# coolo/rl-6-nimmt

Hardware: AMD Instinct MI355X
Metric: env-steps/sec at 65536 concurrent 4-player games, 1/2/4/8 MI355X (higher is better)
Workload: dtype u32; 1 GPU; config2: 65536 x 4-player DrunkHamster self-play per GPU, one episode (10 env-steps) per launch, numpy-MT RNG, int8 obs + actions + rewards + done emitted; games_per_gpu=65536, players=4, env_steps_per_launch=655360, rng=numpy, obs=True, parallelism=dp1 (independent game shards, no data-path collective), launches_per_call=4

## Files before the change

include/sechs.h:

```cpp
#ifndef SECHS_H
#define SECHS_H
#include <stddef.h>
#include <stdint.h>

#ifdef __cplusplus
extern "C" {
#endif

typedef struct sn_env sn_env;

typedef enum {
    SN_OK = 0,
    SN_EINVAL = 1,
    SN_EHIP = 2,
    SN_ENOMEM = 3,
    SN_EUNSUPPORTED = 4,
    SN_ERNG = 5,
} sn_status;

enum {
    SN_RNG_PHILOX = 0,
    SN_RNG_NUMPY_MT = 1,
};

enum { SN_I8 = 1, SN_I16 = 2, SN_I32 = 3, SN_I64 = 4, SN_F32 = 5 };

enum {
    SN_AUTO_RESET = 1,
    SN_NO_SUMMARIES = 2,
};

const char* sn_last_error(void);
const char* sn_version(void);

sn_status sn_create(sn_env** out, int device, int64_t num_games, int num_players, int num_cards, uint64_t seed,
                    uint64_t game_offset, int rng_mode);
sn_status sn_destroy(sn_env* env);
sn_status sn_info(const sn_env* env, int64_t* num_games, int* num_players, int* num_cards, int* rng_mode);

sn_status sn_reset(sn_env* env, const uint8_t* decks, void* stream);

sn_status sn_reset_to(sn_env* env, const int8_t* board, const int8_t* hands, void* stream);

sn_status sn_step(sn_env* env, const int32_t* actions, int32_t* rewards, uint8_t* done, int32_t* invalid, int flags,
                  void* stream);

sn_status sn_rollout(sn_env* env, int steps, int32_t* rewards, uint8_t* done, uint8_t* actions, int8_t* obs,
                     int obs_stride, int flags, void* stream);

sn_status sn_obs(sn_env* env, void* obs, int dtype, int obs_stride, int flags, void* stream);
sn_status sn_hands(sn_env* env, int8_t* hands, void* stream);
sn_status sn_board(sn_env* env, int8_t* board, void* stream);
sn_status sn_scores(sn_env* env, int32_t* scores, void* stream);
sn_status sn_results(sn_env* env, int32_t* sum_results, int32_t* episodes, void* stream);
sn_status sn_clear_results(sn_env* env, void* stream);

sn_status sn_mt_get(sn_env* env, int64_t game, uint32_t* key_host, int32_t* pos_host);
sn_status sn_mt_set(sn_env* env, int64_t game, const uint32_t* key_host, int32_t pos);
sn_status sn_philox_counter(sn_env* env, int64_t game, uint64_t* counter_host);

enum { SN_OPT_RING_WORDS = 1, SN_OPT_CHUNK_STEPS = 2, SN_OPT_PIPELINE = 3, SN_OPT_TIMING = 4, SN_OPT_PIPE_GPW = 5,
       SN_OPT_PIPE_LEAD = 6, SN_OPT_PLAY_SPLIT = 7, SN_OPT_PLAY_QUAD = 8, SN_OPT_TWIST_ROUND = 9,
       SN_OPT_TWIST_EVERY = 10, SN_OPT_PIPE_FUSED = 11, SN_OPT_TWIST_SKIP = 12, SN_OPT_PIPE_DEC = 13,
       SN_OPT_TWIST_DEPTH = 14 };
sn_status sn_set_option(sn_env* env, int option, int value);
sn_status sn_pipe_errors(sn_env* env, uint32_t* count);
sn_status sn_kernel_times(sn_env* env, float* play_ms, float* ahead_ms, int32_t* n);
sn_status sn_kernel_times_dec(sn_env* env, float* play_ms, float* ahead_ms, float* decode_ms, int32_t* n);
sn_status sn_debug_phases(uint64_t* out, int n);
sn_status sn_debug_puct_phases(uint64_t* out, int n);
sn_status sn_debug_pipe_words(sn_env* env, int what, int slot, uint32_t* out);
sn_status sn_debug_failures(uint32_t* count, uint32_t* first_line, int selftest);

sn_status sn_step1(sn_env* env, const int32_t* actions_host, int32_t* out_host, int flags);
sn_status sn_reset1(sn_env* env, const uint32_t* key_host, int32_t pos, uint32_t* key_out_host, int32_t* pos_out,
                    int32_t* out_host, int flags);

sn_status sn_league_config(sn_env* env, int num_agents, int min_players, int max_players);
sn_status sn_league_rollout(sn_env* env, int steps, int32_t* rewards, uint8_t* done, uint8_t* actions, int8_t* obs,
                            int obs_stride, int32_t* records, void* stream);
sn_status sn_league_seats(sn_env* env, uint32_t* out, void* stream);

enum { SN_AGENT_RANDOM = 0, SN_AGENT_MCS = 1, SN_AGENT_EXTERNAL = 2 };
sn_status sn_league_agents(sn_env* env, const int32_t* kinds_host, const int32_t* mc_per_card_host,
                           const int32_t* mc_max_host);
sn_status sn_league_step(sn_env* env, const int32_t* actions, int32_t* rewards, int32_t* played, int32_t* records,
                         int32_t* invalid, int32_t* status, void* stream);
sn_status sn_elo_replay(const int32_t* records_host, int64_t num_games, int max_players, int num_agents, double elo_k,
                        double* elos_host);


sn_status sn_mcs_memorize(sn_env* env, uint32_t* avail, int mcs_num_cards, void* stream);

sn_status sn_mcs_rollouts(sn_env* env, const uint32_t* avail, int rollouts, uint64_t seed, uint32_t decision_step,
                          int32_t* sums, void* stream);
sn_status sn_mcs_rollouts_ex(sn_env* env, const uint32_t* avail, int rollouts, uint64_t seed, uint32_t decision_step,
                             int32_t* sums, int32_t* playouts, void* stream);

sn_status sn_mcs_choose(sn_env* env, const int32_t* sums, int32_t* actions, void* stream);

sn_status sn_mcs_play_exact(sn_env* env, uint32_t mcs_seats, int mc_per_card, int mc_max, int32_t* actions,
                            int32_t* rewards, int32_t* status, void* stream);

sn_status sn_mcs_decide_exact(int device, int64_t num_decisions, int num_players, const int8_t* board,
                              const int8_t* hand, const uint32_t* avail, int mc_per_card, int mc_max,
                              uint32_t* mt_keys, int32_t* mt_pos, int32_t* actions, int32_t* sums, int32_t* counts,
                              void* stream);

typedef struct {
    uint32_t seats_mask;
    int n;
    int puct_root;
    double c_puct;
    uint64_t seed;
    uint32_t step;
    uint32_t rollout;
    const uint32_t* avail;
// ... 56 lines not shown
```

rl-6-nimmt_amd/csrc/sechs_env.hip:

```cpp
#include <hip/hip_runtime.h>

#include <cmath>
#include <cstdio>
#include <cstdlib>
#include <cstring>
#include <new>
#include <string>
#include <type_traits>

#define SECHS_DEBUG_HERE
#include "sechs_state.h"

using namespace sechs;

__global__ void k_seed(DevState s) {
    const int64_t g = (int64_t)blockIdx.x * blockDim.x + threadIdx.x;
    if (g >= s.B) return;
    if (s.rng_mode == RNG_NUMPY_MT) {
        uint32_t* st = s.mt + g * kMtN;
        uint32_t v = (uint32_t)(s.seed + s.game_offset + (uint64_t)g);
        st[0] = v;
        for (int i = 1; i < kMtN; i++) {
            v = 1812433253u * (v ^ (v >> 30)) + (uint32_t)i;
            st[i] = v;
// ... 467 lines not shown
}

enum {
    PH_PROLOGUE = 0, PH_OBS, PH_DRAW, PH_RESOLVE, PH_STORE, PH_DEAL, PH_EPILOGUE, PH_HANDS, PH_APPLY, PH_B1, PH_B2,
    PR_DRAWS, PR_B1, PR_TARGETS, PR_APPLY, PR_HANDS, PR_DRAWS2, PR_B2, PR_STORE, PR_SPARE, PH_N
};
#ifdef SECHS_PHASE_PROF
__device__ unsigned long long g_phase[PH_N + 2];
struct PhaseProf {
    uint64_t t, acc[PH_N];
    __device__ __forceinline__ void start() {
        t = __builtin_readcyclecounter();
#pragma unroll
        for (int k = 0; k < PH_N; k++) acc[k] = 0ull;
    }
    __device__ __forceinline__ void mark(int k) {
        const uint64_t n = __builtin_readcyclecounter();
        acc[k] += n - t;
        t = n;
    }
    __device__ __forceinline__ void flush(int lane, int role = 0) {
        if (lane == 0) {
#pragma unroll
            for (int k = 0; k < PH_N; k++)
                if (acc[k]) atomicAdd(&g_phase[k], (unsigned long long)acc[k]);
            atomicAdd(&g_phase[PH_N + role], 1ull);
        }
    }
};
#else
struct PhaseProf {
    __device__ __forceinline__ void start() {}
    __device__ __forceinline__ void mark(int) {}
    __device__ __forceinline__ void flush(int, int = 0) {}
};
#endif

constexpr int kPlayPrefetch = 2;

struct PlayArgs {
    int steps, flags, obs_stride, wave_lds;
    int ring_lds;
    int pipe_cin, pipe_cout, pipe_t;
    int vec_out;
    const int32_t* actions;
    int32_t* rewards;
    uint8_t* done;
    uint8_t* actions_out;
    int8_t* obs;
    int32_t* invalid;
    int32_t* league_rec;
    int step0;
    int n0;
    int drec0, drec1;
};

template <int N, class R>
struct StreamSrc {
    R& rng;
    ByteBuf& buf;
    uint8_t* deck;
    __device__ __forceinline__ void draws(const Game<N>& G, int, uint32_t kp, bool lg, uint32_t (&idx)[N]) {
        if (lg && !__all(kp == (uint32_t)N)) {
#pragma unroll
            for (int p = 0; p < N; p++) idx[p] = ((uint32_t)p < kp) ? rng_interval(rng, buf, G.n - 1u) : 0u;
        } else {
            rng_draws<N>(rng, buf, G.n - 1u, idx);
        }
    }
    __device__ __forceinline__ uint32_t league(const DevState& s) { return league_draw(rng, buf, s.lg_K, s.lg_lo, s.lg_hi); }
    __device__ __forceinline__ void deal(const DevState& s, Game<N>& G, PhaseProf& pp) {
        shuffle_targets(rng, buf, deck + kDeckStride, s.C);
        pp.mark(PH_DEAL);
        for (int i = 0; i < s.C; i += 4) *(uint32_t*)(deck + i) = (uint32_t)i * 0x01010101u + 0x03020100u;
        shuffle_apply(deck, deck + kDeckStride, s.C);
        pp.mark(PH_APPLY);
        deal_from_deck<N>(deck, s.C, G);
#pragma unroll
        for (int p = 0; p < N; p++) SN_DASSERT(hand_strict(G.hand[p]) && hand_len(G.hand[p]) == (uint32_t)kHand);
    }
};

constexpr int kDecWords = 4 * kDecQuads;

__device__ __forceinline__ uint32_t dec_u16(const uint32_t (&w)[kDecWords], int base, int t) {
    uint32_t v = 0u;
#pragma unroll
    for (int k = 0; k < 5; k++) v = (t >> 1 == k) ? w[base + k] : v;
    return (t & 1) ? (v >> 16) : (v & 0xFFFFu);
}

template <int N>
struct DecSrc {
    uint32_t A[kDecWords];
    uint32_t B1[11];
    int phi;

    __device__ __forceinline__ void load(const DevState& s, const PlayArgs& a, int64_t g, bool cross) {
        phi = a.n0;
        const u32x4* ra = s.drec + (int64_t)a.drec0 * kDecQuads * s.B + g;
#pragma unroll
        for (int q = 0; q < kDecQuads; q++) {
            const u32x4 v = ra[(int64_t)q * s.B];
            A[4 * q] = v.x, A[4 * q + 1] = v.y, A[4 * q + 2] = v.z, A[4 * q + 3] = v.w;
        }
#pragma unroll
        for (int k = 0; k < 11; k++) B1[k] = 0u;
        if (cross) {
            const u32x4* rb = s.drec + (int64_t)a.drec1 * kDecQuads * s.B + g;
#pragma unroll
            for (int q = 0; q < 3; q++) {
                const u32x4 v = rb[(int64_t)q * s.B];
                B1[4 * q] = v.x, B1[4 * q + 1] = v.y, B1[4 * q + 2] = v.z;
                if (q < 2) B1[4 * q + 3] = v.w;
            }
        }
    }
    __device__ __forceinline__ void draws(const Game<N>&, int t, uint32_t, bool, uint32_t (&idx)[N]) {
        const int tau = phi + t;
        uint32_t v;
        if (tau < kHand) {
            v = (tau < kHand - 1) ? dec_u16(A, 6, tau) : 0u;
        } else {
            uint32_t w[kDecWords];
#pragma unroll
            for (int k = 0; k < kDecWords; k++) w[k] = (k < 11) ? B1[k] : 0u;
            v = (tau - kHand < kHand - 1) ? dec_u16(w, 6, tau - kHand) : 0u;
        }
#pragma unroll
        for (int p = 0; p < N; p++) idx[p] = (v >> (4 * p)) & 15u;
    }
    __device__ __forceinline__ uint32_t league(const DevState&) { return 0u; }
    __device__ __forceinline__ void deal(const DevState&, Game<N>& G, PhaseProf&) {
#pragma unroll
        for (int p = 0; p < N; p++) {
            G.hand[p].lo = (uint64_t)A[12 + 3 * p] | ((uint64_t)A[13 + 3 * p] << 32);
            G.hand[p].hi = A[14 + 3 * p];
            G.score[p] = 0;
        }
        const uint32_t rw = A[11];
        const uint32_t r0 = rw & 0xFFu, r1 = (rw >> 8) & 0xFFu, r2 = (rw >> 16) & 0xFFu, r3 = rw >> 24;
        G.b.lo = u32x4{r0, r1, r2, r3};
        G.b.hi = u32x4{meta_row(r0), meta_row(r1), meta_row(r2), meta_row(r3)};
        G.n = kHand;
    }
    __device__ __forceinline__ uint32_t position(int steps) const {
        const int last = phi + steps - 1;
        if (last < kHand) return A[0] + dec_u16(A, 1, last);
        uint32_t w[kDecWords];
#pragma unroll
        for (int k = 0; k < kDecWords; k++) w[k] = (k < 11) ? B1[k] : 0u;
        return w[0] + dec_u16(w, 1, last - kHand);
    }
};

__host__ __device__ constexpr int obs_stage_pieces(int N) { return 3 * N + ((N & 1) ? 0 : 1); }

template <int N, class Src, int GPW = 64, bool LG = false>
__device__ __forceinline__ void play_steps(const DevState& s, const PlayArgs& a, int64_t g, int lane, uint8_t* wave_lds,
                                           Game<N>& G, Src& src, int32_t (&sum_res)[N], int32_t& episodes,
                                           PhaseProf& pp, uint32_t& lg, int t_begin, int t_end) {
    const int64_t B = s.B;
    const bool staged = a.obs && a.obs_stride == 48;
    const int64_t g0 = g - lane;
    const int wave_games = (int)min((int64_t)GPW, B - g0);
    const bool auto_reset = (a.flags & SN_AUTO_RESET) != 0;
    const bool summ = !(a.flags & SN_NO_SUMMARIES);
    int32_t* rew = a.rewards ? a.rewards + ((int64_t)t_begin * B + g) * N : nullptr;
    uint8_t* act = a.actions_out ? a.actions_out + ((int64_t)t_begin * B + g) * N : nullptr;
    uint8_t* dn = a.done ? a.done + (int64_t)t_begin * B + g : nullptr;
    int8_t* ob = a.obs ? a.obs + ((int64_t)t_begin * B + g) * N * a.obs_stride : nullptr;
    for (int t = t_begin; t < t_end; t++) {
        const uint32_t kp = LG ? (lg & 15u) : (uint32_t)N;
        if (ob) {
            uint32_t w2hi;
            const int nobs = LG ? (int)kp : N;
            const GameWords gw = summ ? game_words<true>(nobs, G.b, w2hi) : game_words<false>(nobs, G.b, w2hi);
            if (staged) {
                constexpr int P = obs_stage_pieces(N);
                u32x4* row = (u32x4*)wave_lds + lane * P;
#pragma unroll
                for (int p = 0; p < N; p++) {
                    const Hand& h = G.hand[p];
                    row[3 * p + 0] = u32x4{(uint32_t)h.lo, (uint32_t)(h.lo >> 32), (h.hi & 0xFFFFu) | w2hi, gw.w0};
                    row[3 * p + 1] = gw.a;
                    row[3 * p + 2] = gw.b;
                }
                __builtin_amdgcn_fence(__ATOMIC_SEQ_CST, "wavefront");
                const u32x4* src = (const u32x4*)wave_lds;
                u32x4* dst = (u32x4*)(a.obs + ((int64_t)t * B + g0) * N * 48);
                if (wave_games == GPW) {
                    u32x4 pc[3 * N];
#pragma unroll
                    for (int j = 0; j < 3 * N; j++) {
                        const int c = lane + GPW * j;
                        pc[j] = src[(c / (3 * N)) * P + c % (3 * N)];
                    }
#pragma unroll
                    for (int j = 0; j < 3 * N; j++) {
                        if (SECHS_NT_OBS) __builtin_nontemporal_store(pc[j], &dst[lane + GPW * j]);
                        else dst[lane + GPW * j] = pc[j];
                    }
                } else {
                    const int pieces = wave_games * N * 3;
                    for (int i = lane; i < pieces; i += wave_games) dst[i] = src[(i / (3 * N)) * P + i % (3 * N)];
// ... 87 lines not shown
            if (LG) lg = src.league(s);
            src.deal(s, G, pp);
            if (LG) {
                const uint32_t k2 = lg & 15u;
#pragma unroll
                for (int p = 0; p < N; p++)
                    if ((uint32_t)p >= k2) G.hand[p].lo = ~0ull, G.hand[p].hi = ~0u;
            }
            pp.mark(PH_HANDS);
        }
    }
}

template <int N>
__device__ __forceinline__ void load_results(const DevState& s, int64_t g, int flags, int32_t (&sum_res)[N], int32_t& episodes) {
#pragma unroll
    for (int p = 0; p < N; p++) sum_res[p] = 0;
    episodes = 0;
    if (flags & SN_AUTO_RESET) {
#pragma unroll
        for (int p = 0; p < N; p++) sum_res[p] = s.sum_res[(int64_t)p * s.B + g];
        episodes = s.episodes[g];
    }
}

template <int N>
__device__ __forceinline__ void store_results(const DevState& s, int64_t g, int flags, const int32_t (&sum_res)[N],
                                              int32_t episodes) {
    if (flags & SN_AUTO_RESET) {
#pragma unroll
        for (int p = 0; p < N; p++) s.sum_res[(int64_t)p * s.B + g] = sum_res[p];
        s.episodes[g] = episodes;
    }
}

template <int N, int MODE, int GPW, bool LG = false>
__device__ __forceinline__ void play_body(const DevState& s, const PlayArgs& a, uint8_t* lds_dyn, int tid) {
    const int lane = tid & 63;
    if (GPW < 64 && lane >= GPW) return;
    __builtin_amdgcn_s_setprio(1);
    const int64_t g = ((int64_t)blockIdx.x * (kBlock / 64) + (tid >> 6)) * GPW + lane;
    if (g >= s.B) return;
    uint8_t* wave_lds = lds_dyn + (tid >> 6) * a.wave_lds;
    PhaseProf pp;
    pp.start();
    Game<N> G;
    load_game<N>(s, g, G);
    int32_t sum_res[N], episodes;
    load_results<N>(s, g, a.flags, sum_res, episodes);
    uint32_t lg = LG ? s.lgs[g] : 0u;
    ByteBuf buf;
    if constexpr (MODE == RNG_NUMPY_DEC) {
        DecSrc<N> src;
        src.load(s, a, g, a.n0 + a.steps > kHand);
        pp.mark(PH_PROLOGUE);
        play_steps<N, DecSrc<N>, 64, false>(s, a, g, lane, wave_lds, G, src, sum_res, episodes, pp, lg, 0, a.steps);
        s.pabsc[(int64_t)a.pipe_cout * s.B + g] = src.position(a.steps);
    } else if constexpr (MODE == RNG_NUMPY_PIPE) {
        RingPipe rng;
        rng.load(s, g, buf, wave_lds + a.wave_lds - GPW * a.ring_lds + lane * a.ring_lds, a.pipe_cin, a.pipe_t);
        pp.mark(PH_PROLOGUE);
        StreamSrc<N, RingPipe> src{rng, buf, wave_lds + lane * kDealStride};
        play_steps<N, StreamSrc<N, RingPipe>, GPW, LG>(s, a, g, lane, wave_lds, G, src, sum_res, episodes, pp, lg, 0,
                                                       a.steps);
        s.pabsc[(int64_t)a.pipe_cout * s.B + g] = rng.consumed(buf);
    } else {
        typename RngOf<MODE, kPlayPrefetch>::T rng;
        if constexpr (MODE == RNG_NUMPY_RING || MODE == RNG_NUMPY_RING_HBM) {
            uint8_t* slot = wave_lds + a.wave_lds - 64 * a.ring_lds + lane * a.ring_lds;
            RngOf<MODE, kPlayPrefetch>::load(s, g, rng, buf, slot);
        } else {
            RngOf<MODE, kPlayPrefetch>::load(s, g, rng, buf);
        }
        pp.mark(PH_PROLOGUE);
        using Gen = typename RngOf<MODE, kPlayPrefetch>::T;
        StreamSrc<N, Gen> src{rng, buf, wave_lds + lane * kDealStride};
        play_steps<N, StreamSrc<N, Gen>, 64, LG>(s, a, g, lane, wave_lds, G, src, sum_res, episodes, pp, lg, 0, a.steps);
        RngOf<MODE, kPlayPrefetch>::store(s, g, rng, buf);
    }
    store_game<N>(s, g, G);
    store_results<N>(s, g, a.flags, sum_res, episodes);
    if (LG) s.lgs[g] = lg;
    pp.mark(PH_EPILOGUE);
    pp.flush(lane);
}

template <int N, int MODE, int GPW = 64, bool LG = false>
__global__ __launch_bounds__(kBlock) void k_play(DevState s, PlayArgs a) {
    extern __shared__ __attribute__((aligned(16))) uint8_t lds_dyn[];
    play_body<N, MODE, GPW, LG>(s, a, lds_dyn, (int)threadIdx.x);
}

struct DecArgs {
    int e0, ne, phi0, tpar;
    int cin, cout;
};

constexpr int kDecBlock = 64;
constexpr int kDecLane = kPipeSlot;
static_assert(kDecLane % 8 == 0 && (kDecLane / 8) % 2 == 1 && kDecLane >= 112 + 108, "decoder LDS lane");

template <int N>
__global__ __launch_bounds__(kDecBlock) void k_decode(DevState s, DecArgs d) {
    __shared__ __attribute__((aligned(16))) uint8_t lds[kDecBlock * kDecLane];
    const int lane = threadIdx.x & 63;
    const int64_t g = (int64_t)blockIdx.x * kDecBlock + threadIdx.x;
    if (g >= s.B) return;
    const int64_t B = s.B;
    uint8_t* win = lds + threadIdx.x * kDecLane;
    uint8_t* jslot = win;
    uint8_t* deck = win + 112;
    uint32_t pos = s.pabsc[(int64_t)d.cin * B + g];
    const uint32_t tend = s.ptend[(int64_t)d.tpar * B + g];
    PhaseProf pq;
    pq.start();
    for (int i = 0; i < d.ne; i++) {
        const int phi = (i == 0) ? d.phi0 : 0;
        RingPipe rng;
        ByteBuf buf;
        rng.load_at(s, g, buf, win, pos, tend);
        const uint32_t start = pos;
        uint32_t off[5] = {0u, 0u, 0u, 0u, 0u}, dr[5] = {0u, 0u, 0u, 0u, 0u};
        bool big = false;
#pragma unroll
        for (int t = 0; t < kHand - 1; t++) {
            if (t >= phi) {
                uint32_t idx[N];
                rng_draws<N>(rng, buf, (uint32_t)(kHand - 1 - t), idx);
                uint32_t v = 0u;
#pragma unroll
                for (int p = 0; p < N; p++) v |= idx[p] << (4 * p);
                dr[t >> 1] |= v << (16 * (t & 1));
                const uint32_t o = rng.consumed(buf) - start;
                big = big || o > 0xFFFFu;
                off[t >> 1] |= (o & 0xFFFFu) << (16 * (t & 1));
            }
        }
        pq.mark(PR_DRAWS);
        shuffle_targets(rng, buf, jslot, s.C, kDecLane - 1);
        pos = rng.consumed(buf);
        pq.mark(PR_TARGETS);
// ... 521 lines not shown
    if (num_cards > kMaxCards) return fail(SN_EUNSUPPORTED, "num_cards > 104 (the reference's _card_value asserts card < 104)");
    if (rng_mode != SN_RNG_PHILOX && rng_mode != SN_RNG_NUMPY_MT) return fail(SN_EINVAL, "unknown rng_mode");
    HIP_TRY(hipSetDevice(device));
    sn_env* e = new (std::nothrow) sn_env();
    if (!e) return fail(SN_ENOMEM, "host allocation failed");
    e->device = device;
    if (hipDeviceGetAttribute(&e->cus, hipDeviceAttributeMultiprocessorCount, device) != hipSuccess || e->cus < 1) {
        delete e;
        return fail(SN_EHIP, "cannot query the device's CU count");
    }
    DevState& s = e->s;
    s.B = num_games, s.N = num_players, s.C = num_cards, s.rng_mode = rng_mode;
    s.seed = seed, s.game_offset = game_offset;
    const int64_t B = num_games, N = num_players;
    struct {
        void** p;
        size_t bytes;
    } allocs[] = {
        {(void**)&s.hand, sizeof(uint32_t) * N * 3 * B},   {(void**)&s.row_lo, sizeof(uint32_t) * kRows * B},
        {(void**)&s.row_hi, sizeof(uint32_t) * kRows * B}, {(void**)&s.score, sizeof(int32_t) * N * B},
        {(void**)&s.sum_res, sizeof(int32_t) * N * B},     {(void**)&s.episodes, sizeof(int32_t) * B},
        {(void**)&s.mt_pos, sizeof(uint32_t) * B},         {(void**)&s.ctr, sizeof(uint64_t) * B},
        {(void**)&s.mt, rng_mode == SN_RNG_NUMPY_MT ? sizeof(uint32_t) * kMtN * B : 4},
        {(void**)&s.mt0, sizeof(uint32_t) * kMt0Levels * B},
    };
    for (auto& a : allocs) {
        if (hipMalloc(a.p, a.bytes) != hipSuccess) {
            sn_destroy(e);
            return fail(SN_ENOMEM, "hipMalloc of device state failed");
        }
        (void)hipMemset(*a.p, 0, a.bytes);
    }
    e->opt.chunk_steps = 10;
    e->opt.pipe = 1;
    e->opt.pipe_gpw = 64;
    e->opt.pipe_lead = kPipeLead;
    e->phase = -1;
    e->opt.play_split = 1;
    e->opt.twist_round = 1;
    e->opt.twist_every = 4;
    {
        const char* te = getenv("SECHS_TWIST_EVERY");
        if (te && atoi(te) >= 1 && atoi(te) <= kTwistEveryMax) e->opt.twist_every = atoi(te);
    }
    e->opt.twist_depth = 3;
    {
        const char* td = getenv("SECHS_TWIST_DEPTH");
        if (td && td[0] >= '0' && td[0] <= '0' + kTwistDepthMax && !td[1]) e->opt.twist_depth = td[0] - '0';
    }
    {
        const char* ps = getenv("SECHS_PIPE_SERIAL");
        e->opt.pipe_serial = (ps && ps[0] == '1') ? 1 : 0;
    }
    e->opt.pipe_dec = 1;
    {
        const char* pd = getenv("SECHS_PIPE_DEC");
        if (pd && (pd[0] == '0' || pd[0] == '1')) e->opt.pipe_dec = pd[0] - '0';
    }
    if (rng_mode == SN_RNG_NUMPY_MT) {
        struct {
            void** p;
            size_t bytes;
        } pal[] = {{(void**)&s.pring, (size_t)kPipeRing * B},
                   {(void**)&s.pabsc, sizeof(uint32_t) * (kPipeSlots + 2) * B},
                   {(void**)&s.ptend, sizeof(uint32_t) * kPipeSlots * B}, {(void**)&s.ptp, sizeof(uint32_t) * B},
                   {(void**)&s.perr, sizeof(uint32_t)},
                   {(void**)&s.drec, N <= kSplitMaxPlayers ? sizeof(u32x4) * kDecRecords * kDecQuads * B : 16}};
        for (auto& a : pal) {
            if (hipMalloc(a.p, a.bytes) != hipSuccess) {
                sn_destroy(e);
                return fail(SN_ENOMEM, "hipMalloc of the MT pipeline failed");
            }
            (void)hipMemset(*a.p, 0, a.bytes);
        }
        const char* sf = getenv("SECHS_EV_SYSFENCE");
        const unsigned evf = hipEventDisableTiming | ((sf && sf[0] == '1') ? 0u : (unsigned)hipEventDisableSystemFence);
        if (hipStreamCreateWithFlags(&e->pl.side, hipStreamNonBlocking) != hipSuccess ||
            hipStreamCreateWithFlags(&e->pl.side2, hipStreamNonBlocking) != hipSuccess ||
            hipEventCreateWithFlags(&e->pl.ev_prep2, evf) != hipSuccess ||
            hipEventCreateWithFlags(&e->pl.ev_prep, evf) != hipSuccess ||
            hipEventCreateWithFlags(&e->pl.ev_main, evf) != hipSuccess ||
            hipEventCreateWithFlags(&e->pl.ev_play, evf) != hipSuccess) {
            sn_destroy(e);
            return fail(SN_EHIP, "stream/event creation failed");
        }
        for (int k = 0; k < 2; k++)
            if (hipEventCreateWithFlags(&e->pl.evt[k], evf) != hipSuccess ||
                hipEventCreateWithFlags(&e->pl.evd[k], evf) != hipSuccess) {
                sn_destroy(e);
                return fail(SN_EHIP, "stream/event creation failed");
            }
        if (hipHostMalloc((void**)&e->perr_host, sizeof(uint32_t), hipHostMallocMapped) != hipSuccess ||
            hipHostGetDevicePointer((void**)&e->perr_host_dev, e->perr_host, 0) != hipSuccess) {
            sn_destroy(e);
            return fail(SN_ENOMEM, "pinned overrun mirror allocation failed");
        }
        *e->perr_host = 0u;
    }
    if (rng_mode == SN_RNG_NUMPY_MT) {
        const sn_status r = sn_set_option(e, SN_OPT_RING_WORDS, N <= 4 ? 256 : 512);
        if (r != SN_OK) {
            sn_destroy(e);
            return r;
        }
    }
    hipLaunchKernelGGL(k_seed, dim3(grid_for(B)), dim3(kBlock), 0, 0, s);
// ... 49 lines not shown
    if (!e) return fail(SN_EINVAL, "env is NULL");
    DevState& s = e->s;
    if (sn_pipe_sync(e, 0) != SN_OK) return SN_EHIP;
    switch (option) {
        case SN_OPT_RING_WORDS: {
            if (value < 0 || value > 512 || (value % 64)) return fail(SN_EINVAL, "ring words must be a multiple of 64 in 0..512");
            if (value && s.rng_mode != SN_RNG_NUMPY_MT) return fail(SN_EINVAL, "the ring feeds numpy-compat mode only");
            HIP_TRY(hipSetDevice(e->device));
            HIP_TRY(hipDeviceSynchronize());
            if (s.ring) (void)hipFree(s.ring);
            s.ring = nullptr;
            s.ring_w = 0;
            if (value) {
                if (hipMalloc((void**)&s.ring, (size_t)value * (size_t)s.B) != hipSuccess) return fail(SN_ENOMEM, "ring allocation failed");
                s.ring_w = value;
            }
            return SN_OK;
        }
        case SN_OPT_CHUNK_STEPS:
            if (value < 1) return fail(SN_EINVAL, "chunk steps must be >= 1");
            e->opt.chunk_steps = value;
            return SN_OK;
        case SN_OPT_PIPELINE:
            if (value != 0 && value != 1) return fail(SN_EINVAL, "pipeline must be 0 or 1");
            e->opt.pipe = value;
            return SN_OK;
        case SN_OPT_PIPE_GPW:
            if (value != 32 && value != 64) return fail(SN_EINVAL, "games per wave must be 32 or 64");
            e->opt.pipe_gpw = value;
            return SN_OK;
        case SN_OPT_PLAY_SPLIT:
            if (value < 0 || value > 1) return fail(SN_EINVAL, "play split must be 0 or 1");
            e->opt.play_split = value;
            return SN_OK;
        case SN_OPT_TWIST_EVERY:
            if (value < 1 || value > kTwistEveryMax) return fail(SN_EINVAL, "twist every must be 1 .. 5");
            e->opt.twist_every = value;
            return SN_OK;
        case SN_OPT_TWIST_DEPTH:
            if (value < 0 || value > kTwistDepthMax) return fail(SN_EINVAL, "twist depth must be 0 .. 3");
            e->opt.twist_depth = value;
            return SN_OK;
        case SN_OPT_TWIST_ROUND:
            if (value < 0 || value > 1) return fail(SN_EINVAL, "twist round must be 0 or 1");
            e->opt.twist_round = value;
            return SN_OK;
        case SN_OPT_PLAY_QUAD:
        case SN_OPT_PIPE_FUSED:
            return fail(SN_EUNSUPPORTED, "option removed (k_play_quad / the fused twist measured slower)");
        case SN_OPT_PIPE_DEC:
            if (value < 0 || value > 1) return fail(SN_EINVAL, "pipe dec must be 0 or 1");
            e->opt.pipe_dec = value;
            return SN_OK;
        case SN_OPT_TWIST_SKIP:
            if (value < 0 || value > 1) return fail(SN_EINVAL, "twist skip must be 0 or 1");
            e->opt.twist_skip = value;
            return SN_OK;
        case SN_OPT_PIPE_LEAD:
            if (value < 64 || value > kPipeLead) return fail(SN_EINVAL, "pipe lead must be in 64..600");
            e->opt.pipe_lead = value;
            return SN_OK;
        case SN_OPT_TIMING:
            if (value < 0 || value > 4096) return fail(SN_EINVAL, "timing launches must be in 0..4096");
            HIP_TRY(hipSetDevice(e->device));
            HIP_TRY(hipDeviceSynchronize());
            free_timing(e);
            if (value) {
                e->tev = new hipEvent_t[kTimingEvents * value]();
                e->tev_tw = new int[value]();
                e->tcap = value;
                for (int i = 0; i < kTimingEvents * value; i++) HIP_TRY(hipEventCreate(&e->tev[i]));
            }
            return SN_OK;
        default: return fail(SN_EINVAL, "unknown option");
    }
}

sn_status sn_info(const sn_env* e, int64_t* B, int* N, int* C, int* mode) {
    if (!e) return fail(SN_EINVAL, "env is NULL");
    if (B) *B = e->s.B;
    if (N) *N = e->s.N;
    if (C) *C = e->s.C;
    if (mode) *mode = e->s.rng_mode;
    return SN_OK;
}

sn_status sn_reset(sn_env* e, const uint8_t* decks, void* stream) {
    if (!e) return fail(SN_EINVAL, "env is NULL");
    hipStream_t st = (hipStream_t)stream;
    if (sn_pipe_sync(e, st) != SN_OK) return SN_EHIP;
    const DevState& s = e->s;
    if (s.lg_K) {
        if (decks) return fail(SN_EINVAL, "a tournament handle deals from its own streams (decks must be NULL)");
        if (s.rng_mode == SN_RNG_NUMPY_MT) {
            SN_DISPATCH_N(s.N, {
                if constexpr (NN >= 2 && NN <= kLeagueMaxPlayers)
                    hipLaunchKernelGGL((k_reset<NN, RNG_NUMPY_MT, true>), dim3(grid_for(s.B)), dim3(kBlock), 0, st, s, decks);
            });
        } else {
            SN_DISPATCH_N(s.N, {
                if constexpr (NN >= 2 && NN <= kLeagueMaxPlayers)
                    hipLaunchKernelGGL((k_reset<NN, RNG_PHILOX, true>), dim3(grid_for(s.B)), dim3(kBlock), 0, st, s, decks);
            });
        }
        e->lg_phase = 0;
        e->phase = -1;
// ... 187 lines not shown
    return SN_OK;
}

static sn_status pipe_twist(sn_env* e, uint64_t G, uint64_t p, int64_t e_start, int lead, int ti, hipStream_t st) {
    sn_env::Pipeline& pl = e->pl;
    hipEvent_t* tv = (ti >= 0) ? e->tev + kTimingEvents * ti : nullptr;
    if (e->opt.pipe_serial) HIP_TRY(hipEventRecord(pl.ev_main, st));
    HIP_TRY(hipStreamWaitEvent(pl.side, pl.ev_main, 0));
    if (tv) HIP_TRY(hipEventRecord(tv[2], pl.side));
    const AheadArgs aa{pl.dec ? dec_slot(G - 1) : pabsc_in(p), ptend_slot(G - 1), ptend_slot(G),
                       (e->opt.twist_skip && G >= 1u) ? 0 : lead, e->perr_host_dev, -1, e->opt.twist_depth};
    if (const sn_status r = launch_ahead(e->s, false, e->opt.twist_round, aa, pl.side); r != SN_OK) return r;
    if (tv) HIP_TRY(hipEventRecord(tv[3], pl.side));
    if (pl.dec) {
        const int64_t target = e_start + 2 * pl.K + 1;
        if (e->opt.pipe_serial || G == 0u) HIP_TRY(hipStreamWaitEvent(pl.side2, pl.ev_main, 0));
        if (G >= 1u) HIP_TRY(hipStreamWaitEvent(pl.side2, pl.evt[ptend_slot(G - 1)], 0));
        if (tv) HIP_TRY(hipEventRecord(tv[4], pl.side2));
        const int ne = target > pl.dec_next ? (int)(target - pl.dec_next) : 0;
        const sn_status r = dec_launch(e, pl.dec_next, ne, 0, ptend_slot(G - 1), dec_slot(G - 1), dec_slot(G), pl.side2);
        if (r != SN_OK) return r;
        pl.dec_next = max(pl.dec_next, target);
        if (tv) {
            HIP_TRY(hipEventRecord(tv[5], pl.side2));
            e->tev_tw[ti] |= 2;
        }
        HIP_TRY(hipEventRecord(pl.evd[ptend_slot(G)], pl.side2));
    }
    HIP_TRY(hipEventRecord(pl.evt[ptend_slot(G)], pl.side));
    HIP_TRY(hipEventRecord(pl.ev_prep, pl.side));
    pl.tw_out = ptend_slot(G);
    return SN_OK;
}

static sn_status launch_pipe(sn_env* e, PlayArgs a, LdsPlan plan, hipStream_t st) {
    const DevState& s = e->s;
    sn_env::Pipeline& pl = e->pl;
    const int gpw = e->opt.pipe_gpw, K = e->opt.twist_every;
    const bool dec = dec_ok(e, a);
    const int mode = dec ? RNG_NUMPY_DEC : RNG_NUMPY_PIPE;
    apply_plan(a, dec ? lds_plan(s.N, obs_staged(a.obs, a.obs_stride), RNG_NUMPY_DEC) : plan);
    if (pl.valid && (pl.K != K || (pl.dec != 0) != dec)) {
        if (const sn_status r = sn_pipe_sync(e, st); r != SN_OK) return r;
    }
    const int lead = dec ? min(e->opt.pipe_lead * (K + 1), kPipeRing - kMtN) : e->opt.pipe_lead * K;
    static_assert(kPipeLeadMax <= kPipeRing - kMtN, "the decode-ahead lead is never capped by the ring");
    if (!pl.valid) {
        if (const sn_status r = pipe_start(e, K, dec, lead, st); r != SN_OK) return r;
    } else {
        HIP_TRY(hipStreamWaitEvent(st, pl.ev_play, 0));
    }
    const int chunk = min(e->opt.chunk_steps, (s.lg_K > 8) ? 5 : pipe_max_chunk(s.N));
    int phase = dec ? e->phase : 0;
    for (int t0 = 0; t0 < a.steps; t0 += chunk) {
        PlayArgs c = slice_steps(a, t0, min(chunk, a.steps - t0), s.B, s.N);
        const uint64_t p = pl.launches, G = p / (uint64_t)K;
        const bool first = (p % (uint64_t)K) == 0u;
        c.pipe_cin = pabsc_in(p), c.pipe_cout = pabsc_out(p);
        c.pipe_t = ptend_slot(G - 1);
        if (dec) {
            c.n0 = phase;
            c.drec0 = dec_record(pl.dec_e), c.drec1 = dec_record(pl.dec_e + 1);
        }
        if (first && G >= 1u) HIP_TRY(hipStreamWaitEvent(st, (dec ? pl.evd : pl.evt)[ptend_slot(G - 1)], 0));
        if (first && !e->opt.pipe_serial) HIP_TRY(hipEventRecord(pl.ev_main, st));
        const int ti = (e->tn < e->tcap) ? e->tn++ : -1;
        hipEvent_t* tv = (ti >= 0) ? e->tev + kTimingEvents * ti : nullptr;
        if (tv) e->tev_tw[ti] = first ? 1 : 0;
        if (tv) HIP_TRY(hipEventRecord(tv[0], st));
        if (const sn_status r = launch_play_mode(s, c, mode, gpw, st); r != SN_OK) return r;
        const int64_t e_start = pl.dec_e;
        if (dec) {
            phase += c.steps;
            if (phase >= kHand) phase -= kHand, pl.dec_e++;
        }
        if (tv) HIP_TRY(hipEventRecord(tv[1], st));
        if (first) {
            if (const sn_status r = pipe_twist(e, G, p, e_start, lead, ti, st); r != SN_OK) return r;
        }
        pl.pl_cout = c.pipe_cout;
        pl.launches++;
    }
    HIP_TRY(hipEventRecord(pl.ev_play, st));
    return SN_OK;
}

static sn_status launch_play(sn_env* e, PlayArgs a, hipStream_t st) {
    const DevState& s = e->s;
    const bool numpy = s.rng_mode == SN_RNG_NUMPY_MT;
    a.vec_out = ((((uintptr_t)a.rewards) & 15) == 0) && ((((uintptr_t)a.actions_out) & 3) == 0);
    if (s.lg_K) {
        if (a.actions) return fail(SN_EUNSUPPORTED, "a tournament handle plays in-kernel DrunkHamster seats only (sn_rollout)");
        if (!(a.flags & SN_AUTO_RESET)) return fail(SN_EINVAL, "a tournament handle rolls out with SN_AUTO_RESET");
    }
    if (numpy && !a.actions && (e->opt.pipe || s.lg_K)) {
        const LdsPlan plan = lds_plan(s.N, obs_staged(a.obs, a.obs_stride), RNG_NUMPY_PIPE, e->opt.pipe_gpw);
        const bool fits = block_lds(plan) <= (size_t)kLdsBytes;
        if (s.lg_K && (!e->opt.pipe || e->opt.pipe_gpw != 64 || !fits))
            return fail(SN_EUNSUPPORTED, "tournament rollouts need the pipelined numpy-MT path (64 games per wave)");
        if (fits) return launch_pipe(e, a, plan, st);
    }
    if (const sn_status r = sn_pipe_sync(e, st); r != SN_OK) return r;
    const bool ring = numpy && !a.actions && s.ring_w > 0;
    const int chunk = ring ? e->opt.chunk_steps : a.steps;
    for (int t0 = 0; t0 < a.steps; t0 += chunk) {
        const sn_status r = launch_play_one(e, slice_steps(a, t0, min(chunk, a.steps - t0), s.B, s.N), st);
        if (r != SN_OK) return r;
    }
    return SN_OK;
}


sn_status sn_step(sn_env* e, const int32_t* actions, int32_t* rewards, uint8_t* done, int32_t* invalid, int flags,
                  void* stream) {
    if (!e) return fail(SN_EINVAL, "env is NULL");
    if (e->s.lg_K) return fail(SN_EUNSUPPORTED, "a tournament handle plays whole games with sn_league_rollout");
    e->phase = -1;
    PlayArgs a{};
    a.steps = 1;
    a.flags = flags;
    a.actions = actions;
    a.rewards = rewards;
    a.done = done;
    a.invalid = invalid;
    return launch_play(e, a, (hipStream_t)stream);
}

sn_status sn_rollout(sn_env* e, int steps, int32_t* rewards, uint8_t* done, uint8_t* actions, int8_t* obs,
                     int obs_stride, int flags, void* stream) {
    if (!e) return fail(SN_EINVAL, "env is NULL");
    if (steps < 0) return fail(SN_EINVAL, "steps must be >= 0");
    const int L = (flags & SN_NO_SUMMARIES) ? 35 : 47;
    if (obs && (obs_stride < L || (obs_stride & 3))) return fail(SN_EINVAL, "obs_stride must be a multiple of 4 and >= obs length");
    if (check_obs_align(obs, obs_stride) != SN_OK) return SN_EINVAL;
// ... 387 lines not shown
```

rl-6-nimmt_amd/csrc/sechs_state.h:

```cpp
#pragma once
#include <hip/hip_runtime.h>

#include <string>

#include "../../include/sechs.h"
#include "sechs_device.h"

namespace sechs {

struct DevState {
    int64_t B;
    int N, C, rng_mode, pad_;
    uint64_t seed, game_offset;
    uint32_t* hand;
    uint32_t* row_lo;
    uint32_t* row_hi;
    int32_t* score;
    int32_t* sum_res;
    int32_t* episodes;
    uint32_t* mt;
    uint32_t* mt_pos;
    uint64_t* ctr;
    uint32_t* mt0;
    u32x4* ring;
// ... 667 lines not shown
        for (int i = 12; i < nw; i++) d[i] = 0u;
    }
}


sn_status set_error(sn_status st, const std::string& msg);
inline unsigned grid_for(int64_t n) { return (unsigned)((n + kBlock - 1) / kBlock); }

#define HIP_TRY(expr)                                                                                    \
    do {                                                                                                 \
        hipError_t e_ = (expr);                                                                          \
        if (e_ != hipSuccess) return ::sechs::set_error(SN_EHIP, std::string(#expr ": ") + hipGetErrorString(e_)); \
    } while (0)

#ifdef SECHS_DEV_ONLY_N
#define SN_DISPATCH_N(N_, BODY)                                                              \
    if ((N_) == SECHS_DEV_ONLY_N) {                                                          \
        constexpr int NN = SECHS_DEV_ONLY_N;                                                 \
        BODY;                                                                                \
    } else                                                                                   \
        return ::sechs::set_error(SN_EUNSUPPORTED, "development build: one player count only");
#else
#define SN_DISPATCH_N(N_, BODY)                                                          \
    switch (N_) {                                                                        \
        case 1: { constexpr int NN = 1; BODY; } break;                                   \
        case 2: { constexpr int NN = 2; BODY; } break;                                   \
        case 3: { constexpr int NN = 3; BODY; } break;                                   \
        case 4: { constexpr int NN = 4; BODY; } break;                                   \
        case 5: { constexpr int NN = 5; BODY; } break;                                   \
        case 6: { constexpr int NN = 6; BODY; } break;                                   \
        case 7: { constexpr int NN = 7; BODY; } break;                                   \
        case 8: { constexpr int NN = 8; BODY; } break;                                   \
        case 9: { constexpr int NN = 9; BODY; } break;                                   \
        case 10: { constexpr int NN = 10; BODY; } break;                                 \
        default: return ::sechs::set_error(SN_EINVAL, "num_players out of range");      \
    }
#endif

}

struct sn_env {
    int device;
    int cus;
    int lg_phase;
    int lg_kind[16];
    int lg_mpc[16], lg_mmax[16];
    int phase;
    struct Options {
        int chunk_steps;
        int pipe;
        int pipe_gpw;
        int pipe_lead;
        int pipe_dec;
        int pipe_serial;
        int play_split;
        int twist_every;
        int twist_round;
        int twist_depth;
        int twist_skip;
    } opt;
    sechs::DevState s;
    struct Pipeline {
        int valid;
        int K, dec;
        uint64_t launches;
        int tw_out;
        int pl_cout;
        int64_t dec_e;
        int64_t dec_next;
        hipStream_t side, side2;
        hipEvent_t evt[2];
        hipEvent_t evd[2], ev_prep2;
        hipEvent_t ev_prep, ev_main, ev_play;
    } pl;
    uint32_t* perr_host;
    uint32_t* perr_host_dev;
    uint32_t* hbuf;
    uint32_t* hbuf_dev;
    hipEvent_t* tev;
    int* tev_tw;
    int tcap, tn;
};

extern "C" sn_status sn_pipe_sync(sn_env* e, hipStream_t st);
```

rl-6-nimmt_amd/rl_6_nimmt/_native.py:

```python
import ctypes
import os

import torch

_PKG_ROOT = os.path.dirname(os.path.dirname(os.path.abspath(__file__)))
LIB_PATH = os.environ.get("SECHS_LIB", os.path.join(_PKG_ROOT, "libsechs.so"))

SN_OK, SN_EINVAL, SN_EHIP, SN_ENOMEM, SN_EUNSUPPORTED, SN_ERNG = 0, 1, 2, 3, 4, 5
SN_RNG_PHILOX, SN_RNG_NUMPY_MT = 0, 1
SN_I8, SN_I16, SN_I32, SN_I64, SN_F32 = 1, 2, 3, 4, 5
SN_AUTO_RESET, SN_NO_SUMMARIES = 1, 2
SN_OPT_RING_WORDS, SN_OPT_CHUNK_STEPS, SN_OPT_PIPELINE, SN_OPT_TIMING, SN_OPT_PIPE_GPW, SN_OPT_PIPE_LEAD = 1, 2, 3, 4, 5, 6
SN_OPT_PLAY_SPLIT = 7
SN_OPT_TWIST_ROUND = 9
SN_OPT_TWIST_EVERY = 10
SN_OPT_TWIST_SKIP = 12
SN_OPT_PIPE_DEC = 13
SN_OPT_TWIST_DEPTH = 14
SN_AGENT_RANDOM, SN_AGENT_MCS, SN_AGENT_EXTERNAL = 0, 1, 2

class SnPuct(ctypes.Structure):

    _fields_ = [
        ("seats_mask", ctypes.c_uint32),
        ("n", ctypes.c_int),
        ("puct_root", ctypes.c_int),
        ("c_puct", ctypes.c_double),
        ("seed", ctypes.c_uint64),
        ("step", ctypes.c_uint32),
        ("rollout", ctypes.c_uint32),
        ("avail", ctypes.c_void_p),
        ("rollouts", ctypes.c_void_p),
        ("stats", ctypes.c_void_p),
        ("hist", ctypes.c_void_p),
        ("root_probs", ctypes.c_void_p),
        ("step_dev", ctypes.c_void_p),
        ("dec_list", ctypes.c_void_p),
        ("num_dec", ctypes.c_int64),
        ("logit_stride", ctypes.c_int32),
        ("logit_bf16", ctypes.c_int32),
    ]


_P = ctypes.c_void_p
_I = ctypes.c_int
_I64 = ctypes.c_int64
_U64 = ctypes.c_uint64
SIGNATURES = {
    "sn_last_error": ([], ctypes.c_char_p),
    "sn_version": ([], ctypes.c_char_p),
    "sn_create": ([ctypes.POINTER(_P), _I, _I64, _I, _I, _U64, _U64, _I], _I),
    "sn_destroy": ([_P], _I),
    "sn_info": ([_P, _P, _P, _P, _P], _I),
    "sn_reset": ([_P, _P, _P], _I),
    "sn_reset_to": ([_P, _P, _P, _P], _I),
    "sn_step": ([_P, _P, _P, _P, _P, _I, _P], _I),
    "sn_rollout": ([_P, _I, _P, _P, _P, _P, _I, _I, _P], _I),
    "sn_obs": ([_P, _P, _I, _I, _I, _P], _I),
    "sn_hands": ([_P, _P, _P], _I),
    "sn_board": ([_P, _P, _P], _I),
    "sn_scores": ([_P, _P, _P], _I),
    "sn_results": ([_P, _P, _P, _P], _I),
    "sn_clear_results": ([_P, _P], _I),
    "sn_mt_get": ([_P, _I64, _P, _P], _I),
    "sn_mt_set": ([_P, _I64, _P, ctypes.c_int32], _I),
    "sn_philox_counter": ([_P, _I64, _P], _I),
    "sn_set_option": ([_P, _I, _I], _I),
    "sn_pipe_errors": ([_P, _P], _I),
    "sn_kernel_times": ([_P, _P, _P, _P], _I),
    "sn_kernel_times_dec": ([_P, _P, _P, _P, _P], _I),
    "sn_debug_phases": ([_P, _I], _I),
# ... 98 lines not shown
```

rl-6-nimmt_amd/rl_6_nimmt/vec_env.py:

```python
import ctypes

import numpy as np
import torch

from . import _native as nat

RNG_MODES = {"philox": nat.SN_RNG_PHILOX, "numpy": nat.SN_RNG_NUMPY_MT}
ROWS, THRESHOLD, HAND = 4, 6, 10


def obs_length(include_summaries=True):
    return 10 + 1 + (3 * ROWS if include_summaries else 0) + ROWS * THRESHOLD


class VecSechsNimmtEnv:
    def __init__(self, num_games, num_players=4, num_cards=104, seed=0, game_offset=0, rng="numpy", device=None,
                 include_summaries=True):
        nat.require_gpu()
        if rng not in RNG_MODES:
            raise ValueError(f"rng must be one of {sorted(RNG_MODES)}")
        if device is None:
            idx = torch.cuda.current_device()
        else:
            d = torch.device(device)
# ... 71 lines not shown
            if want_actions:
                out["actions"] = self._empty((T, B, N), torch.uint8)
            if want_obs:
                out["obs"] = self._empty((T, B, N, stride), torch.int8)
        if "obs" in out:
            stride = out["obs"].shape[-1]
        nat.check(
            nat.lib().sn_rollout(self._h, T, nat.ptr(out.get("rewards")), nat.ptr(out.get("done")),
                                 nat.ptr(out.get("actions")), nat.ptr(out.get("obs")), stride,
                                 self._flags(True), self._stream()),
            "sn_rollout",
        )
        if check and self.rng == "numpy":
            n = self.pipe_errors()
            if n:
                raise nat.PipeOverrunError(f"sn_rollout: {n} pipelined MT19937 draws ran past the twisted words")
        return out

    _DT = {torch.int8: nat.SN_I8, torch.int16: nat.SN_I16, torch.int32: nat.SN_I32, torch.int64: nat.SN_I64,
           torch.float32: nat.SN_F32}

    def obs(self, dtype=torch.int8, stride=None):
        stride = stride or self.obs_len
        o = self._empty((self.num_games, self.num_players, stride), dtype)
        nat.check(nat.lib().sn_obs(self._h, nat.ptr(o), self._DT[dtype], stride, self._flags(), self._stream()), "sn_obs")
        return o

    def hands(self):
        h = self._empty((self.num_games, self.num_players, HAND), torch.int8)
        nat.check(nat.lib().sn_hands(self._h, nat.ptr(h), self._stream()), "sn_hands")
        return h

    def board(self):
        b = self._empty((self.num_games, ROWS, THRESHOLD), torch.int8)
        nat.check(nat.lib().sn_board(self._h, nat.ptr(b), self._stream()), "sn_board")
        return b

    def scores(self):
        s = self._empty((self.num_games, self.num_players), torch.int32)
        nat.check(nat.lib().sn_scores(self._h, nat.ptr(s), self._stream()), "sn_scores")
        return s

    def results(self):
        s = self._empty((self.num_games, self.num_players), torch.int32)
        e = self._empty((self.num_games,), torch.int32)
        nat.check(nat.lib().sn_results(self._h, nat.ptr(s), nat.ptr(e), self._stream()), "sn_results")
        return s, e

    def clear_results(self):
        nat.check(nat.lib().sn_clear_results(self._h, self._stream()), "sn_clear_results")

    def set_option(self, ring_words=None, chunk_steps=None, pipeline=None, pipe_gpw=None, pipe_lead=None,
                   play_split=None, twist_round=None, twist_every=None, twist_skip=None, pipe_dec=None,
                   twist_depth=None):
        if pipe_lead is not None:
            nat.check(nat.lib().sn_set_option(self._h, nat.SN_OPT_PIPE_LEAD, int(pipe_lead)), "sn_set_option")
        if pipe_gpw is not None:
            nat.check(nat.lib().sn_set_option(self._h, nat.SN_OPT_PIPE_GPW, int(pipe_gpw)), "sn_set_option")
        if play_split is not None:
            nat.check(nat.lib().sn_set_option(self._h, nat.SN_OPT_PLAY_SPLIT, int(play_split)), "sn_set_option")
        if twist_every is not None:
            nat.check(nat.lib().sn_set_option(self._h, nat.SN_OPT_TWIST_EVERY, int(twist_every)), "sn_set_option")
        if twist_round is not None:
            nat.check(nat.lib().sn_set_option(self._h, nat.SN_OPT_TWIST_ROUND, int(twist_round)), "sn_set_option")
        if twist_depth is not None:
            nat.check(nat.lib().sn_set_option(self._h, nat.SN_OPT_TWIST_DEPTH, int(twist_depth)), "sn_set_option")
        if pipe_dec is not None:
            nat.check(nat.lib().sn_set_option(self._h, nat.SN_OPT_PIPE_DEC, int(pipe_dec)), "sn_set_option")
        if twist_skip is not None:
            nat.check(nat.lib().sn_set_option(self._h, nat.SN_OPT_TWIST_SKIP, int(twist_skip)), "sn_set_option")
        if pipeline is not None:
            nat.check(nat.lib().sn_set_option(self._h, nat.SN_OPT_PIPELINE, int(bool(pipeline))), "sn_set_option")
        if ring_words is not None:
            nat.check(nat.lib().sn_set_option(self._h, nat.SN_OPT_RING_WORDS, int(ring_words)), "sn_set_option")
        if chunk_steps is not None:
            nat.check(nat.lib().sn_set_option(self._h, nat.SN_OPT_CHUNK_STEPS, int(chunk_steps)), "sn_set_option")

    def time_kernels(self, launches):
        nat.check(nat.lib().sn_set_option(self._h, nat.SN_OPT_TIMING, int(launches)), "sn_set_option")

    def kernel_times(self, with_decode=False):
        a, b, c, n = ctypes.c_float(), ctypes.c_float(), ctypes.c_float(), ctypes.c_int32()
        nat.check(nat.lib().sn_kernel_times_dec(self._h, ctypes.byref(a), ctypes.byref(b), ctypes.byref(c),
                                                ctypes.byref(n)), "sn_kernel_times_dec")
        return (a.value, b.value, c.value, n.value) if with_decode else (a.value, b.value, n.value)

    def pipe_errors(self):
        c = ctypes.c_uint32()
        nat.check(nat.lib().sn_pipe_errors(self._h, ctypes.byref(c)), "sn_pipe_errors")
        return c.value

    def get_mt_state(self, game=0):
        key = np.zeros(624, dtype=np.uint32)
        pos = ctypes.c_int32()
        torch.cuda.current_stream(self.device).synchronize()
        nat.check(nat.lib().sn_mt_get(self._h, game, key.ctypes.data_as(ctypes.c_void_p), ctypes.byref(pos)), "sn_mt_get")
        return key, int(pos.value)

    def set_mt_state(self, key, pos, game=0):
        key = np.ascontiguousarray(key, dtype=np.uint32)
        assert key.shape == (624,)
        torch.cuda.current_stream(self.device).synchronize()
        nat.check(nat.lib().sn_mt_set(self._h, game, key.ctypes.data_as(ctypes.c_void_p), int(pos)), "sn_mt_set")

    def philox_counter(self, game=0):
        c = ctypes.c_uint64()
        torch.cuda.current_stream(self.device).synchronize()
        nat.check(nat.lib().sn_philox_counter(self._h, game, ctypes.byref(c)), "sn_philox_counter")
        return int(c.value)
```

Baseline: 11.42 billion env-steps/s.

## Fuse consecutive decoded play chunks into one launch with rolling record fetch

In the decoded-RNG pipeline path, the host now groups several step chunks within one twist group into a single k_play launch, and the pipeline bookkeeping advances by the number of merged chunks. DecSrc no longer preloads two records with a cross-boundary buffer. It keeps one record and fetches the next slot whenever a round ends mid-launch. The play kernel also gets a waves-per-EU attribute, which for the max-player decoded variant lets the compiler use more registers. The aim is to cut launch count and per-launch prologue cost and to shrink register pressure, at the price of less interleaving with the twist/decode kernels and possible occupancy loss.

```diff
diff --git a/include/sechs.h b/include/sechs.h
--- a/include/sechs.h
+++ b/include/sechs.h
@@ -62,7 +62,7 @@
 enum { SN_OPT_RING_WORDS = 1, SN_OPT_CHUNK_STEPS = 2, SN_OPT_PIPELINE = 3, SN_OPT_TIMING = 4, SN_OPT_PIPE_GPW = 5,
        SN_OPT_PIPE_LEAD = 6, SN_OPT_PLAY_SPLIT = 7, SN_OPT_PLAY_QUAD = 8, SN_OPT_TWIST_ROUND = 9,
        SN_OPT_TWIST_EVERY = 10, SN_OPT_PIPE_FUSED = 11, SN_OPT_TWIST_SKIP = 12, SN_OPT_PIPE_DEC = 13,
-       SN_OPT_TWIST_DEPTH = 14 };
+       SN_OPT_TWIST_DEPTH = 14, SN_OPT_PLAY_GROUP = 15 };
 sn_status sn_set_option(sn_env* env, int option, int value);
 sn_status sn_pipe_errors(sn_env* env, uint32_t* count);
 sn_status sn_kernel_times(sn_env* env, float* play_ms, float* ahead_ms, int32_t* n);
diff --git a/rl-6-nimmt_amd/csrc/sechs_env.hip b/rl-6-nimmt_amd/csrc/sechs_env.hip
--- a/rl-6-nimmt_amd/csrc/sechs_env.hip
+++ b/rl-6-nimmt_amd/csrc/sechs_env.hip
@@ -543,7 +543,7 @@
     int32_t* league_rec;
     int step0;
     int n0;
-    int drec0, drec1;
+    int drec0;
 };
 
 template <int N, class R>
@@ -584,40 +584,29 @@
 template <int N>
 struct DecSrc {
     uint32_t A[kDecWords];
-    uint32_t B1[11];
-    int phi;
-
-    __device__ __forceinline__ void load(const DevState& s, const PlayArgs& a, int64_t g, bool cross) {
-        phi = a.n0;
-        const u32x4* ra = s.drec + (int64_t)a.drec0 * kDecQuads * s.B + g;
+    const u32x4* rec;
+    int64_t B;
+    int slot;
+    int base;
+    int end;
+
+    __device__ __forceinline__ void fetch() {
+        const u32x4* ra = rec + (int64_t)slot * kDecQuads * B;
 #pragma unroll
         for (int q = 0; q < kDecQuads; q++) {
-            const u32x4 v = ra[(int64_t)q * s.B];
+            const u32x4 v = ra[(int64_t)q * B];
             A[4 * q] = v.x, A[4 * q + 1] = v.y, A[4 * q + 2] = v.z, A[4 * q + 3] = v.w;
         }
-#pragma unroll
-        for (int k = 0; k < 11; k++) B1[k] = 0u;
-        if (cross) {
-            const u32x4* rb = s.drec + (int64_t)a.drec1 * kDecQuads * s.B + g;
-#pragma unroll
-            for (int q = 0; q < 3; q++) {
-                const u32x4 v = rb[(int64_t)q * s.B];
-                B1[4 * q] = v.x, B1[4 * q + 1] = v.y, B1[4 * q + 2] = v.z;
-                if (q < 2) B1[4 * q + 3] = v.w;
-            }
-        }
+    }
+    __device__ __forceinline__ void load(const DevState& s, const PlayArgs& a, int64_t g) {
+        rec = s.drec + g, B = s.B;
+        slot = a.drec0, base = -a.n0, end = a.steps;
+        fetch();
     }
     __device__ __forceinline__ void draws(const Game<N>&, int t, uint32_t, bool, uint32_t (&idx)[N]) {
-        const int tau = phi + t;
-        uint32_t v;
-        if (tau < kHand) {
-            v = (tau < kHand - 1) ? dec_u16(A, 6, tau) : 0u;
-        } else {
-            uint32_t w[kDecWords];
-#pragma unroll
-            for (int k = 0; k < kDecWords; k++) w[k] = (k < 11) ? B1[k] : 0u;
-            v = (tau - kHand < kHand - 1) ? dec_u16(w, 6, tau - kHand) : 0u;
-        }
+        const int tau = t - base;
+        SN_DASSERT(tau >= 0 && tau < kHand);
+        const uint32_t v = (tau < kHand - 1) ? dec_u16(A, 6, tau) : 0u;
 #pragma unroll
         for (int p = 0; p < N; p++) idx[p] = (v >> (4 * p)) & 15u;
     }
@@ -634,14 +623,18 @@
         G.b.lo = u32x4{r0, r1, r2, r3};
         G.b.hi = u32x4{meta_row(r0), meta_row(r1), meta_row(r2), meta_row(r3)};
         G.n = kHand;
-    }
-    __device__ __forceinline__ uint32_t position(int steps) const {
-        const int last = phi + steps - 1;
-        if (last < kHand) return A[0] + dec_u16(A, 1, last);
-        uint32_t w[kDecWords];
-#pragma unroll
-        for (int k = 0; k < kDecWords; k++) w[k] = (k < 11) ? B1[k] : 0u;
-        return w[0] + dec_u16(w, 1, last - kHand);
+        if (base + kHand < end) {
+            base += kHand;
+            slot = (slot + 1 == kDecRecords) ? 0 : slot + 1;
+            fetch();
+#pragma unroll
+            for (int k = 0; k < kDecWords; k++) asm volatile("" : "+v"(A[k]));
+        }
+    }
+    __device__ __forceinline__ uint32_t position() const {
+        const int last = end - 1 - base;
+        SN_DASSERT(last >= 0 && last < kHand);
+        return A[0] + dec_u16(A, 1, last);
     }
 };
 
@@ -835,10 +828,10 @@
     ByteBuf buf;
     if constexpr (MODE == RNG_NUMPY_DEC) {
         DecSrc<N> src;
-        src.load(s, a, g, a.n0 + a.steps > kHand);
+        src.load(s, a, g);
         pp.mark(PH_PROLOGUE);
         play_steps<N, DecSrc<N>, 64, false>(s, a, g, lane, wave_lds, G, src, sum_res, episodes, pp, lg, 0, a.steps);
-        s.pabsc[(int64_t)a.pipe_cout * s.B + g] = src.position(a.steps);
+        s.pabsc[(int64_t)a.pipe_cout * s.B + g] = src.position();
     } else if constexpr (MODE == RNG_NUMPY_PIPE) {
         RingPipe rng;
         rng.load(s, g, buf, wave_lds + a.wave_lds - GPW * a.ring_lds + lane * a.ring_lds, a.pipe_cin, a.pipe_t);
@@ -869,7 +862,9 @@
 }
 
 template <int N, int MODE, int GPW = 64, bool LG = false>
-__global__ __launch_bounds__(kBlock) void k_play(DevState s, PlayArgs a) {
+__global__ __launch_bounds__(kBlock)
+__attribute__((amdgpu_waves_per_eu(1, (MODE == RNG_NUMPY_DEC && N == kSplitMaxPlayers) ? 1 : 8)))
+void k_play(DevState s, PlayArgs a) {
     extern __shared__ __attribute__((aligned(16))) uint8_t lds_dyn[];
     play_body<N, MODE, GPW, LG>(s, a, lds_dyn, (int)threadIdx.x);
 }
@@ -1497,6 +1492,11 @@
         const char* ps = getenv("SECHS_PIPE_SERIAL");
         e->opt.pipe_serial = (ps && ps[0] == '1') ? 1 : 0;
     }
+    e->opt.play_group = 1;
+    {
+        const char* pg = getenv("SECHS_PLAY_GROUP");
+        if (pg && (pg[0] == '0' || pg[0] == '1') && !pg[1]) e->opt.play_group = pg[0] - '0';
+    }
     e->opt.pipe_dec = 1;
     {
         const char* pd = getenv("SECHS_PIPE_DEC");
@@ -1652,6 +1652,10 @@
             if (value < 0 || value > 1) return fail(SN_EINVAL, "pipe dec must be 0 or 1");
             e->opt.pipe_dec = value;
             return SN_OK;
+        case SN_OPT_PLAY_GROUP:
+            if (value < 0 || value > 1) return fail(SN_EINVAL, "play group must be 0 or 1");
+            e->opt.play_group = value;
+            return SN_OK;
         case SN_OPT_TWIST_SKIP:
             if (value < 0 || value > 1) return fail(SN_EINVAL, "twist skip must be 0 or 1");
             e->opt.twist_skip = value;
@@ -1945,15 +1949,17 @@
     }
     const int chunk = min(e->opt.chunk_steps, (s.lg_K > 8) ? 5 : pipe_max_chunk(s.N));
     int phase = dec ? e->phase : 0;
-    for (int t0 = 0; t0 < a.steps; t0 += chunk) {
-        PlayArgs c = slice_steps(a, t0, min(chunk, a.steps - t0), s.B, s.N);
+    const bool fuse = dec && e->opt.play_group;
+    for (int t0 = 0, m = 1; t0 < a.steps; t0 += m * chunk) {
         const uint64_t p = pl.launches, G = p / (uint64_t)K;
         const bool first = (p % (uint64_t)K) == 0u;
-        c.pipe_cin = pabsc_in(p), c.pipe_cout = pabsc_out(p);
+        m = fuse ? (int)min((int64_t)(a.steps - t0 + chunk - 1) / chunk, (int64_t)K - (int64_t)(p % (uint64_t)K)) : 1;
+        PlayArgs c = slice_steps(a, t0, min(m * chunk, a.steps - t0), s.B, s.N);
+        c.pipe_cin = pabsc_in(p), c.pipe_cout = pabsc_out(p + (uint64_t)m - 1u);
         c.pipe_t = ptend_slot(G - 1);
         if (dec) {
             c.n0 = phase;
-            c.drec0 = dec_record(pl.dec_e), c.drec1 = dec_record(pl.dec_e + 1);
+            c.drec0 = dec_record(pl.dec_e);
         }
         if (first && G >= 1u) HIP_TRY(hipStreamWaitEvent(st, (dec ? pl.evd : pl.evt)[ptend_slot(G - 1)], 0));
         if (first && !e->opt.pipe_serial) HIP_TRY(hipEventRecord(pl.ev_main, st));
@@ -1965,14 +1971,14 @@
         const int64_t e_start = pl.dec_e;
         if (dec) {
             phase += c.steps;
-            if (phase >= kHand) phase -= kHand, pl.dec_e++;
+            pl.dec_e += phase / kHand, phase %= kHand;
         }
         if (tv) HIP_TRY(hipEventRecord(tv[1], st));
         if (first) {
             if (const sn_status r = pipe_twist(e, G, p, e_start, lead, ti, st); r != SN_OK) return r;
         }
         pl.pl_cout = c.pipe_cout;
-        pl.launches++;
+        pl.launches += (uint64_t)m;
     }
     HIP_TRY(hipEventRecord(pl.ev_play, st));
     return SN_OK;
diff --git a/rl-6-nimmt_amd/csrc/sechs_state.h b/rl-6-nimmt_amd/csrc/sechs_state.h
--- a/rl-6-nimmt_amd/csrc/sechs_state.h
+++ b/rl-6-nimmt_amd/csrc/sechs_state.h
@@ -743,6 +743,7 @@
         int pipe_gpw;
         int pipe_lead;
         int pipe_dec;
+        int play_group;
         int pipe_serial;
         int play_split;
         int twist_every;
diff --git a/rl-6-nimmt_amd/rl_6_nimmt/_native.py b/rl-6-nimmt_amd/rl_6_nimmt/_native.py
--- a/rl-6-nimmt_amd/rl_6_nimmt/_native.py
+++ b/rl-6-nimmt_amd/rl_6_nimmt/_native.py
@@ -17,6 +17,7 @@
 SN_OPT_TWIST_SKIP = 12
 SN_OPT_PIPE_DEC = 13
 SN_OPT_TWIST_DEPTH = 14
+SN_OPT_PLAY_GROUP = 15
 SN_AGENT_RANDOM, SN_AGENT_MCS, SN_AGENT_EXTERNAL = 0, 1, 2
 
 class SnPuct(ctypes.Structure):
diff --git a/rl-6-nimmt_amd/rl_6_nimmt/vec_env.py b/rl-6-nimmt_amd/rl_6_nimmt/vec_env.py
--- a/rl-6-nimmt_amd/rl_6_nimmt/vec_env.py
+++ b/rl-6-nimmt_amd/rl_6_nimmt/vec_env.py
@@ -147,7 +147,7 @@
 
     def set_option(self, ring_words=None, chunk_steps=None, pipeline=None, pipe_gpw=None, pipe_lead=None,
                    play_split=None, twist_round=None, twist_every=None, twist_skip=None, pipe_dec=None,
-                   twist_depth=None):
+                   twist_depth=None, play_group=None):
         if pipe_lead is not None:
             nat.check(nat.lib().sn_set_option(self._h, nat.SN_OPT_PIPE_LEAD, int(pipe_lead)), "sn_set_option")
         if pipe_gpw is not None:
@@ -160,6 +160,8 @@
             nat.check(nat.lib().sn_set_option(self._h, nat.SN_OPT_TWIST_ROUND, int(twist_round)), "sn_set_option")
         if twist_depth is not None:
             nat.check(nat.lib().sn_set_option(self._h, nat.SN_OPT_TWIST_DEPTH, int(twist_depth)), "sn_set_option")
+        if play_group is not None:
+            nat.check(nat.lib().sn_set_option(self._h, nat.SN_OPT_PLAY_GROUP, int(play_group)), "sn_set_option")
         if pipe_dec is not None:
             nat.check(nat.lib().sn_set_option(self._h, nat.SN_OPT_PIPE_DEC, int(pipe_dec)), "sn_set_option")
         if twist_skip is not None:
```

New measurement: 11.72 billion env-steps/s (median of 6 runs). +2.6%, better.
